# Elensil/Facet_Graph_Convolution

Measured on AMD Instinct MI355X. Metric: facets/sec (fwd+bwd) on 100k-facet mesh, higher is better.
Workload: dtype f32; 1 GPU; c2: torus 250x200 quads = 100000 facets per GPU (N0=122224 padded nodes), full graph U-Net + MLP: rotate + forward + angular loss + backward + Adam, fp32, hipGraph replay; parallelism=single GPU

## Files before the change

### facet_graph_convolution_amd/csrc/fgc_conv_bwd.hip

```cpp
#include <stdio.h>
#include <stdlib.h>
#include <string.h>

#include <algorithm>
#include <type_traits>

#include "fgc_conv_bwd.h"
#include "fgc_conv_narrow.h"
#include "fgc_conv_pair.h"
#include "fgc_gemm_tn.h"
#include "fgc_reduce.h"
#include "fgc_split.h"

namespace fgc {

__device__ __forceinline__ float slope_from_y(float y, float alpha) { return y > 0.f ? 1.f : (y < 0.f ? alpha : 0.f); }

__device__ __forceinline__ float pool4_grad_term(const float* __restrict__ y, const float* __restrict__ pool_y,
                                                 const float* __restrict__ pool_dy, int r, int col, int cout, int bf16) {
    const size_t pi = (size_t)(r >> 2) * cout + col;
    const float m = ld_act(pool_y, pi, bf16);
    const size_t b = (size_t)(r & ~3) * cout + col;
    float ne = 0.f;
#pragma unroll
// ... 752 lines not shown
                    }
                    dq[n0 + nn] += t0 + t1;
                }
            };
            products(0, bxa);
            if (!LONG) {
                products(H, bxb);
            } else {
                gather(H, bxa);
                products(H, bxa);
#pragma unroll
                for (int nn = 0; nn < NPW; ++nn) {
                    if (dn[nn] <= 16) continue;
                    const int node = wave * NPW + nn;
                    const int e = min(16 + lr, dn[nn] - 1);
                    const int row = __float_as_int(s.qbuf[(size_t)node * qnode_stride(QS) + e * QLD + 9]);
                    const unsigned off = __umul24((unsigned)row, rowbytes) + laneoff;
                    const f32x4 x0 = __builtin_bit_cast(f32x4, __builtin_amdgcn_raw_buffer_load_b128(rsrc, off, 0, 0));
                    const f32x4 x1 = __builtin_bit_cast(f32x4, __builtin_amdgcn_raw_buffer_load_b128(rsrc, off + 64u, 0, 0));
                    const float* zr = s.ztile + (size_t)node * ZSTRIDE + mrow * KC + 4 * lq;
                    const f32x4 a0 = *reinterpret_cast<const f32x4*>(zr);
                    const f32x4 a1 = *reinterpret_cast<const f32x4*>(zr + 16);
                    f32x4 u0 = f32x4{0.f, 0.f, 0.f, 0.f}, u1 = f32x4{0.f, 0.f, 0.f, 0.f};
#pragma unroll
                    for (int t = 0; t < 4; ++t) {
                        u0 = __builtin_amdgcn_mfma_f32_16x16x4f32(a0[t], x0[t], u0, 0, 0, 0);
                        u1 = __builtin_amdgcn_mfma_f32_16x16x4f32(a1[t], x1[t], u1, 0, 0, 0);
                    }
                    dq_hi[nn] += u0 + u1;
                }
            }
        }

#pragma unroll
        for (int nn = 0; nn < NPW; ++nn) {
            const int node = wave * NPW + nn;
            const int i = tile0 + node;
            const int d = dn[nn];
            if (i >= p.n) continue;
            if (d <= ebase) {
                if (sweep == 0 && lr == 0 && lq < 3)
                    *reinterpret_cast<f32x4*>(lp.dag + (size_t)i * FGC_AG_LD + 4 * lq) = f32x4{0.f, 0.f, 0.f, 0.f};
                continue;
            }
            const int e0 = s.deg[TILE + 4 + node];
            f32x4 da = f32x4{0.f, 0.f, 0.f, 0.f};
            const int ntile = (FGC_KO1 & 32) ? 0 : ((LONG && d > 16) ? 2 : 1);
            for (int et = 0; et < ntile; ++et) {
                const int edge = ebase + 16 * et + lr;
                const bool ok = edge < d;
                const float* qr = s.qbuf + (size_t)node * qnode_stride(QS) + min(edge, d - 1) * QLD;
                f32x4 q = f32x4{0.f, 0.f, 0.f, 0.f};
                if (lq < 2) q = *reinterpret_cast<const f32x4*>(qr + 4 * lq);
                else if (lq == 2) q[0] = qr[8];
                f32x4 g = (LONG && et == 1) ? dq_hi[LONG ? nn : 0] : dq[nn];
                if (lq == 2) { g[1] = 0.f; g[2] = 0.f; g[3] = 0.f; }
                if (lq == 3) g = f32x4{0.f, 0.f, 0.f, 0.f};
                float dot = q[0] * g[0] + q[1] * g[1] + q[2] * g[2] + q[3] * g[3];
                dot += __shfl_xor(dot, 16);
                dot += __shfl_xor(dot, 32);
                f32x4 dl;
#pragma unroll
                for (int t = 0; t < 4; ++t) dl[t] = ok ? q[t] * (g[t] - dot) : 0.f;
                if (!(FGC_KO1 & 64) && ok && lq < 3) *reinterpret_cast<f32x4*>(lp.dl + (size_t)(e0 + edge) * FGC_DL_LD + 4 * lq) = dl;
                da += dl;
            }
// ... 977 lines not shown
```

### facet_graph_convolution_amd/csrc/fgc_conv_w8.hip

```cpp
#include <stdlib.h>

#include "fgc_conv_w8.h"

namespace fgc {

#ifndef FGC_KO
#define FGC_KO 0
#endif
constexpr int W8_THREADS = 512;
constexpr int W8_LPN = 16;
typedef float f32x2 __attribute__((ext_vector_type(2)));

__device__ __forceinline__ f32x2 load_chunk2(const CoreParams& p, int row, int cbase) {
    const float* ptr = cbase < p.c0 ? p.src0 + (size_t)row * p.c0 + cbase
                                    : p.src1 + (size_t)row * p.c1 + (cbase - p.c0);
    f32x2 v = {0.f, 0.f};
    if (cbase < p.cg) v = *reinterpret_cast<const f32x2*>(ptr);
    return v;
}

template <int N, bool BF>
__device__ __forceinline__ void edge_batch(__amdgpu_buffer_rsrc_t rsrc, unsigned rowbytes, unsigned laneoff,
                                           const float* qk, f32x2 (&z)[FGC_M]) {
    f32x2 q89[N], xv[N];
// ... 27 lines not shown
#pragma unroll
    for (int t = 0; t < N; ++t) rid[t] = (unsigned)__float_as_int(qb[(T0 + t) * QLD + 9]);
#pragma unroll
    for (int t = 0; t < N; ++t) {
        const unsigned off = __umul24(rid[t], rowbytes) + laneoff;
        if (FGC_KO & 16) { raw[T0 + t] = f32x2{__uint_as_float(off), 1.f}; continue; }
        if constexpr (BF) raw[T0 + t][0] = __builtin_bit_cast(float, __builtin_amdgcn_raw_buffer_load_b32(rsrc, off, 0, 0));
        else raw[T0 + t] = __builtin_bit_cast(f32x2, __builtin_amdgcn_raw_buffer_load_b64(rsrc, off, 0, 0));
    }
}
template <int T0, int N, bool BF>
__device__ __forceinline__ void fma_rows(const float* qb, const f32x2 (&raw)[16], f32x2 (&z)[FGC_M]) {
#pragma unroll
    for (int t = 0; t < N; ++t) {
        const float* qk = qb + (T0 + t) * QLD;
        f32x2 xv;
        if constexpr (BF) xv = bf2_to_f2(__builtin_bit_cast(unsigned, raw[T0 + t][0]));
        else xv = raw[T0 + t];
        if (FGC_KO & 2) { z[t % FGC_M] += xv; continue; }
        const f32x4 q0 = *reinterpret_cast<const f32x4*>(qk);
        const f32x4 q1 = *reinterpret_cast<const f32x4*>(qk + 4);
        const float q8 = qk[8];
        z[0] += q0[0] * xv; z[1] += q0[1] * xv; z[2] += q0[2] * xv; z[3] += q0[3] * xv;
        z[4] += q1[0] * xv; z[5] += q1[1] * xv; z[6] += q1[2] * xv; z[7] += q1[3] * xv;
        z[8] += q8 * xv;
    }
}
__device__ __forceinline__ void wave_lds_sync() {
    __builtin_amdgcn_fence(__ATOMIC_RELEASE, "wavefront");
    __builtin_amdgcn_wave_barrier();
    __builtin_amdgcn_fence(__ATOMIC_ACQUIRE, "wavefront");
}

template <bool DATA, bool FAST, int QS, bool BF = false, int NT = 32, bool EROW = false>
__global__ __launch_bounds__(NT * 16, 4) void conv_w8_kernel(CoreParams p, FwdEpilogue fe, DataEpilogue de) {
    static_assert(!BF || FAST, "the bf16 form exists for the fast shapes only");
    static_assert(!EROW || (DATA && FAST), "rows by edge id: the data-gradient kernel's fast shapes");
    static_assert(NT == 32 || (NT == 16 && FAST && QS == 16), "half tiles: the pipelined 16-slot form only");
    constexpr int TILE = NT, RT = NT / 16, NW = NT / 4, LW = NT == 32 ? 3 : 2, W8_THREADS = NT * 16;
    extern __shared__ __attribute__((aligned(16))) char smem_raw[];
    const Smem s = carve(smem_raw, BF ? ZSTRIDE_BF / 2 : ZSTRIDE, QS, NT);
    constexpr int SPL = QS / 16 + (QS % 16 ? 1 : 0);
    constexpr bool PIPE = FAST && QS == 16;
    auto dag_slot = [&](int nd, int m) { return s.qbuf + (size_t)nd * qnode_stride(QS) + m * QLD + 10; };
    int tile0;
    if constexpr (NT == 32) {
        tile0 = block_tile0(p);
    } else {
        const int h = xcd_tile(blockIdx.x, gridDim.x);
        tile0 = (p.tile_list ? p.tile_list[h >> 1] : (h >> 1)) * 32 + (h & 1) * 16;
    }
    const int tid = threadIdx.x;
    const int node = tid >> 4, kl = tid & 15;
    const int wave = tid >> 6, lane = tid & 63, lr = lane & 15, lq = lane >> 4;
    const int nct = p.npad >> 4;
    const int nsh = 31 - __builtin_clz(nct);
    const int kparts = NW >> nsh;
    const int ct = __builtin_amdgcn_readfirstlane(wave & (nct - 1));
    const int kpart = __builtin_amdgcn_readfirstlane(wave >> nsh);
    constexpr int UPP = BF ? KPASS / 32 : KPASS / 16;
    const int u0 = __builtin_amdgcn_readfirstlane((UPP * kpart) >> (LW - nsh));
    const int u1 = __builtin_amdgcn_readfirstlane((UPP * (kpart + 1)) >> (LW - nsh));
    const __amdgpu_buffer_rsrc_t w_rs = __builtin_amdgcn_make_buffer_rsrc(const_cast<float*>(p.Wp), 0, -1, 0x00020000);
    const unsigned w_lane = BF ? (unsigned)((ct * 64 + lane) * 16) : (unsigned)((lq * p.npad + ct * 16 + lr) * 16);
    const unsigned w_unit = BF ? (unsigned)(nct * 1024) : (unsigned)(p.npad * 64);
    auto loadw = [&](int pass, int u) {
        const int uu = min(u, u1 - 1);
        if (FGC_KO & 512) return u32x4{(unsigned)uu, (unsigned)pass, 0x3f800000u, 0x3f000000u};
        return __builtin_bit_cast(u32x4, __builtin_amdgcn_raw_buffer_load_b128(w_rs, w_lane, (unsigned)(pass * UPP + uu) * w_unit, 0));
    };
    f32x2 xa[16];
    const float* qb = s.qbuf + (size_t)node * qnode_stride(QS);
    auto issue = [&](int pass, int dw) {
        constexpr unsigned ESZ = BF ? 2u : 4u;
        const bool first = pass * KC < p.c0;
        const float* base = first ? p.src0 : p.src1;
// ... 109 lines not shown
#pragma unroll
            for (int m = 0; m < FGC_M; ++m) {
                l[m] = __builtin_amdgcn_exp2f(fmaf(l[m], 1.4426950408889634f, nmx));
                sum += l[m];
            }
            const float inv = 1.0f / sum;
            float* q = s.qbuf + (size_t)node * qnode_stride(QS) + k * QLD;
            *reinterpret_cast<f32x4*>(q) = f32x4{l[0] * inv, l[1] * inv, l[2] * inv, l[3] * inv};
            *reinterpret_cast<f32x4*>(q + 4) = f32x4{l[4] * inv, l[5] * inv, l[6] * inv, l[7] * inv};
            q[8] = l[8] * inv;
            if (!PIPE) q[9] = __int_as_float(er[t]);
            if (DATA && !(FGC_KO & 256)) {
                const __amdgpu_buffer_rsrc_t dl_rs = __builtin_amdgcn_make_buffer_rsrc(const_cast<float*>(de.dl), 0, -1, 0x00020000);
                const unsigned dof = __umul24((unsigned)(EROW ? er[t] : p.eid[e0 + k]), FGC_DL_LD * 4u);
                const f32x4 d0 = __builtin_bit_cast(f32x4, __builtin_amdgcn_raw_buffer_load_b128(dl_rs, dof, 0, 0));
                const f32x4 d1 = __builtin_bit_cast(f32x4, __builtin_amdgcn_raw_buffer_load_b128(dl_rs, dof + 16u, 0, 0));
                dgsum[0] += d0[0]; dgsum[1] += d0[1]; dgsum[2] += d0[2]; dgsum[3] += d0[3];
                dgsum[4] += d1[0]; dgsum[5] += d1[1]; dgsum[6] += d1[2]; dgsum[7] += d1[3];
                dgsum[8] += __builtin_bit_cast(float, __builtin_amdgcn_raw_buffer_load_b32(dl_rs, dof + 32u, 0, 0));
            }
        }
        if (DATA) {
#pragma unroll
            for (int m = 0; m < FGC_M; ++m) {
                float v = dgsum[m];
                FGC_ROW16_SUM(v);
                dgsum[m] = v;
            }
            if (kl == 0) {
                if (i < p.n) {
                    const float da[FGC_M] = {da0[0], da0[1], da0[2], da0[3], da1[0], da1[1], da1[2], da1[3], da8};
#pragma unroll
                    for (int m = 0; m < FGC_M; ++m) *reinterpret_cast<f32x2*>(dag_slot(node, m)) = f32x2{da[m], dgsum[m]};
                    float* o = de.dag + (size_t)i * FGC_AG_LD + 12;
                    *reinterpret_cast<f32x4*>(o) = f32x4{dgsum[0], dgsum[1], dgsum[2], dgsum[3]};
                    *reinterpret_cast<f32x4*>(o + 4) = f32x4{dgsum[4], dgsum[5], dgsum[6], dgsum[7]};
                    *reinterpret_cast<f32x4*>(o + 8) = f32x4{dgsum[8], 0.f, 0.f, 0.f};
                    if constexpr (BF) {
                        u32x2* rt = reinterpret_cast<u32x2*>(reinterpret_cast<unsigned short*>(de.r) + (size_t)i * de.rld +
                                                             (FGC_M * p.cg));
                        rt[0] = f4_to_bf4(f32x4{da[0], da[1], da[2], da[3]});
                        rt[1] = f4_to_bf4(f32x4{da[4], da[5], da[6], da[7]});
                        rt[2] = f4_to_bf4(f32x4{da[8], 0.f, 0.f, 0.f});
                        rt[3] = f4_to_bf4(f32x4{dgsum[0], dgsum[1], dgsum[2], dgsum[3]});
                        rt[4] = f4_to_bf4(f32x4{dgsum[4], dgsum[5], dgsum[6], dgsum[7]});
                        rt[5] = f4_to_bf4(f32x4{dgsum[8], 0.f, 0.f, 0.f});
                    } else {
                    float* rt = de.r + (size_t)i * de.rld + (FGC_M * p.cg);
                    *reinterpret_cast<f32x4*>(rt) = f32x4{da[0], da[1], da[2], da[3]};
                    *reinterpret_cast<f32x4*>(rt + 4) = f32x4{da[4], da[5], da[6], da[7]};
                    *reinterpret_cast<f32x4*>(rt + 8) = f32x4{da[8], 0.f, 0.f, 0.f};
                    *reinterpret_cast<f32x4*>(rt + 12) = f32x4{dgsum[0], dgsum[1], dgsum[2], dgsum[3]};
                    *reinterpret_cast<f32x4*>(rt + 16) = f32x4{dgsum[4], dgsum[5], dgsum[6], dgsum[7]};
                    *reinterpret_cast<f32x4*>(rt + 20) = f32x4{dgsum[8], 0.f, 0.f, 0.f};
                    }
                }
            }
        }
    }
    if constexpr (PIPE) wave_lds_sync();
    else __syncthreads();

    f32x4 acc[RT];
#pragma unroll
    for (int r = 0; r < RT; ++r) acc[r] = f32x4{0.f, 0.f, 0.f, 0.f};
    const bool want_gemm = !DATA || de.dx0 != nullptr;

    const int cl = kl;
    const int d = s.deg[node];
    auto do_pass = [&](int pass) {
        f32x2 z[FGC_M];
#pragma unroll
        for (int m = 0; m < FGC_M; ++m) z[m] = f32x2{0.f, 0.f};
        const int cbase = pass * KC + 2 * cl;
        if constexpr (PIPE) {
            fma_rows<0, 8, BF>(qb, xa, z);
            if (dwave > 8) fma_rows<8, 4, BF>(qb, xa, z);
            if (dwave > 12) fma_rows<12, 1, BF>(qb, xa, z);
            if (dwave > 13) fma_rows<13, 1, BF>(qb, xa, z);
            if (dwave > 14) fma_rows<14, 2, BF>(qb, xa, z);
            if (pass + 1 < p.passes) issue(pass + 1, dwave);
        } else if (FAST) {
            const bool first = pass * KC < p.c0;
            const float* base = first ? p.src0 : p.src1;
            constexpr unsigned ESZ = BF ? 2u : 4u;
            const unsigned rowbytes = (unsigned)(first ? p.c0 : p.c1) * ESZ;
            const unsigned laneoff = (unsigned)(first ? cbase : cbase - p.c0) * ESZ;
            const __amdgpu_buffer_rsrc_t rsrc = __builtin_amdgcn_make_buffer_rsrc(const_cast<float*>(base), 0, -1, 0x00020000);
            int k0 = 0;
            for (; k0 + 8 <= dwave; k0 += 8) edge_batch<8, BF>(rsrc, rowbytes, laneoff, qb + k0 * QLD, z);
            const int rem = dwave - k0;
            if (rem > 4) {
                if (rem > 6) edge_batch<8, BF>(rsrc, rowbytes, laneoff, qb + k0 * QLD, z);
                else edge_batch<6, BF>(rsrc, rowbytes, laneoff, qb + k0 * QLD, z);
            } else if (rem > 0) {
                if (rem > 2) edge_batch<4, BF>(rsrc, rowbytes, laneoff, qb + k0 * QLD, z);
                else edge_batch<2, BF>(rsrc, rowbytes, laneoff, qb + k0 * QLD, z);
            }
        } else
        for (int k0 = 0; k0 < d; k0 += RB) {
            f32x2 xv[RB];
#pragma unroll
            for (int t = 0; t < RB; ++t) {
                xv[t] = f32x2{0.f, 0.f};
                if (k0 + t < d) xv[t] = load_chunk2(p, __float_as_int(qb[(k0 + t) * QLD + 9]), cbase);
            }
#pragma unroll
            for (int t = 0; t < RB; ++t) {
                if (k0 + t < d) {
                    const float* q = qb + (k0 + t) * QLD;
                    const f32x4 q0 = *reinterpret_cast<const f32x4*>(q);
                    const f32x4 q1 = *reinterpret_cast<const f32x4*>(q + 4);
                    const float q8 = q[8];
                    z[0] += q0[0] * xv[t]; z[1] += q0[1] * xv[t]; z[2] += q0[2] * xv[t]; z[3] += q0[3] * xv[t];
                    z[4] += q1[0] * xv[t]; z[5] += q1[1] * xv[t]; z[6] += q1[2] * xv[t]; z[7] += q1[3] * xv[t];
                    z[8] += q8 * xv[t];
                }
            }
        }        if (DATA) {
            const int j = tile0 + node;
            if (!(FGC_KO & 128) && j < p.n && cbase < p.cg) {
                if constexpr (BF) {
                    unsigned* rr = reinterpret_cast<unsigned*>(reinterpret_cast<unsigned short*>(de.r) + (size_t)j * de.rld + cbase);
#pragma unroll
                    for (int m = 0; m < FGC_M; ++m) rr[(m * p.cg) >> 1] = f2_to_bf2(z[m][0], z[m][1]);
                } else {
                float* rr = de.r + (size_t)j * de.rld + cbase;
#pragma unroll
                for (int m = 0; m < FGC_M; ++m) *reinterpret_cast<f32x2*>(rr + m * p.cg) = z[m];
                }
            }
            if (!want_gemm) return;
        }
        auto gphase32 = [&](int gl, int gh, int gz) {
        auto loadw = [&](int pass_, int u) {
            const int uu = min(u, gh - 1);
            if (FGC_KO & 512) return u32x4{(unsigned)uu, (unsigned)pass_, 0x3f800000u, 0x3f000000u};
            return __builtin_bit_cast(u32x4, __builtin_amdgcn_raw_buffer_load_b128(w_rs, w_lane, (unsigned)(pass_ * UPP + uu) * w_unit, 0));
        };
        auto loada = [&](int g, f32x4 (&a)[RT]) {
            const int gg = min(g, gh - 1) - gz;
#pragma unroll
            for (int r = 0; r < RT; ++r)
                a[r] = *reinterpret_cast<const f32x4*>(s.ztile + (size_t)(r * 16 + lr) * ZSTRIDE + gg * 16 + lq * 4);
        };
        auto mm = [&](const f32x4 (&a)[RT], const u32x4& bw) {
            const f32x4 b = __builtin_bit_cast(f32x4, bw);
#pragma unroll
            for (int t = 0; t < 4; ++t)
#pragma unroll
                for (int r = 0; r < RT; ++r) {
                    if (FGC_KO & 1) asm volatile("" ::"v"(a[r][t]), "v"(b[t]));
// ... 9 lines not shown
                mm(a0, b0);
                b0 = loadw(pass, g + 4);
                loada(g + 2, a0);
                mm(a1, b1);
                b1 = loadw(pass, g + 5);
                loada(g + 3, a1);
                mm(a0, b2);
                b2 = loadw(pass, g + 6);
                loada(g + 4, a0);
                mm(a1, b3);
                b3 = loadw(pass, g + 7);
            }
            if (g < gh) {
                loada(g + 1, a1);
                mm(a0, b0);
            }
            if (g + 1 < gh) {
                loada(g + 2, a0);
                mm(a1, b1);
            }
            if (g + 2 < gh) mm(a0, b2);
        };
        if (pass > 0) __syncthreads();
        if constexpr (BF) {
            unsigned* zr = reinterpret_cast<unsigned*>(s.ztile) + (size_t)node * (ZSTRIDE_BF / 2) + cl;
#pragma unroll
            for (int m = 0; m < FGC_M; ++m) zr[m * (KC / 2)] = f2_to_bf2(z[m][0], z[m][1]);
        } else {
            float* zr = s.ztile + (size_t)node * ZSTRIDE + 2 * cl;
#pragma unroll
            for (int m = 0; m < FGC_M; ++m) *reinterpret_cast<f32x2*>(zr + m * KC) = z[m];
        }
        __syncthreads();
        if (FGC_KO & 8) return;
        const char* zb = reinterpret_cast<const char*>(s.ztile);
        auto mmb = [&](int ks, const u32x4& b) {
#pragma unroll
            for (int r = 0; r < RT; ++r) {
                const u32x4 a = *reinterpret_cast<const u32x4*>(zb + (size_t)(r * 16 + lr) * (ZSTRIDE_BF * 2) + ks * 64 + lq * 16);
                acc[r] = __builtin_amdgcn_mfma_f32_16x16x32_bf16(__builtin_bit_cast(bf16x8, a), __builtin_bit_cast(bf16x8, b),
                                                                acc[r], 0, 0, 0);
            }
        };
        if constexpr (BF) {
            int ks = u0;
            u32x4 b0 = loadw(pass, ks), b1 = loadw(pass, ks + 1);
            for (; ks + 2 <= u1; ks += 2) {
                mmb(ks, b0);
                b0 = loadw(pass, ks + 2);
                mmb(ks + 1, b1);
                b1 = loadw(pass, ks + 3);
            }
            if (ks < u1) mmb(ks, b0);
        } else {
            gphase32(u0, u1, 0);
        }
    };
    for (int pass = 0; pass < p.passes; ++pass) do_pass(pass);
    if (!want_gemm) return;
    if (FGC_KO & 32) { if (acc[0][0] == 123.f && acc[RT - 1][3] == 5.f) s.ztile[tid] = acc[0][1]; return; }
    __syncthreads();
    const int oldd = p.npad + 4;
    float* otile = s.ztile;
    {
        float* base = otile + (size_t)kpart * TILE * oldd;
#pragma unroll
        for (int r = 0; r < RT; ++r)
#pragma unroll
            for (int t = 0; t < 4; ++t) base[(size_t)(r * 16 + lq * 4 + t) * oldd + ct * 16 + lr] = acc[r][t];
    }
    __syncthreads();
    if (!DATA) {
        const int osh = 31 - __builtin_clz(p.nout);
        const bool pow2 = FAST && (p.nout & (p.nout - 1)) == 0;
        const int o = pow2 ? (tid & (p.nout - 1)) : tid % p.nout, pstep = pow2 ? (W8_THREADS >> osh) : W8_THREADS / p.nout;
        const float bias_o = fe.bias[o];
        for (int pr = tid < pstep * p.nout ? (pow2 ? tid >> osh : tid / p.nout) : TILE; pr < TILE / 4; pr += pstep) {
            float mx = -INFINITY;
            bool any = false;
            const size_t ybase = (size_t)(tile0 + pr * 4) * p.nout + o;
#pragma unroll
            for (int q = 0; q < 4; ++q) {
                const int row = pr * 4 + q;
                const int i = tile0 + row;
                if (i >= p.n) continue;
                float val = 0.f;
                for (int kp = 0; kp < kparts; ++kp) val += otile[((size_t)kp * TILE + row) * oldd + o];
                const int dd = s.deg[row];
                val *= __int_as_float(s.deg[TILE + 4 + row]);
                if (!fe.bias_mask || dd > 0) val += bias_o;
                if (fe.act) val = fmaxf(val, 0.f) - fe.alpha * fmaxf(-val, 0.f);
                st_act(fe.y, ybase + (size_t)(q * p.nout), val, BF);
// ... 11 lines not shown
        float uc[FGC_M], vc[FGC_M];
#pragma unroll
        for (int m = 0; m < FGC_M; ++m) {
            uc[m] = de.u[m * de.cin + c];
            vc[m] = de.v[m * de.cin + c];
        }
        for (int sr = tid < sstep * de.cin ? (pow2 ? tid >> csh : tid / de.cin) : nsrc; sr < nsrc; sr += sstep) {
            float val = 0.f;
            bool any = false;
            for (int q = 0; q < group; ++q) {
                const int row = sr * group + q;
                if (tile0 + row >= p.n) continue;
                any = true;
                float g = 0.f;
                for (int kp = 0; kp < kparts; ++kp) g += otile[((size_t)kp * TILE + row) * oldd + c];
#pragma unroll
                for (int m = 0; m < FGC_M; ++m) {
                    const f32x2 dd = *reinterpret_cast<const f32x2*>(dag_slot(row, m));
                    g = fmaf(dd[0], uc[m], g);
                    g = fmaf(dd[1], vc[m], g);
                }
                val += g;
            }
            if (!any) continue;
            const size_t srow = (size_t)((tile0 >> de.shiftf) + sr);
            if (c < de.c0f) {
                const size_t o = srow * de.c0f + c;
                st_act(de.dx0, o, de.acc0 ? ld_act(de.dx0, o, BF) + val : val, BF);
            } else if (de.dx1) {
                const size_t o = srow * de.c1f + (c - de.c0f);
                st_act(de.dx1, o, de.acc1 ? ld_act(de.dx1, o, BF) + val : val, BF);
            }
        }
    }
}

bool w8_supported(const CoreParams& p, int max_deg) {
    if (opt(OPT_NO_W8) == 1) return false;
    const int nct = p.npad >> 4;
    if (!(nct == 1 || nct == 2 || nct == 4 || nct == 8)) return false;
    if (max_deg <= 0 || max_deg > KMAX) return false;
    if (p.kc != 32) return false;
    if ((p.c0 & 1) || (p.c1 & 1)) return false;
    if (((uintptr_t)p.src0 & 7) || (p.src1 && ((uintptr_t)p.src1 & 7))) return false;
    return true;
}

static bool w8_fast(const CoreParams& p) {
    if (opt(OPT_NO_W8FAST) == 1) return false;
    return p.cg % 32 == 0 && (p.c1 == 0 || p.c0 % 32 == 0) && (size_t)p.n * 4 * 128 < 0xFFFFFFFFull;
}

static bool w8_half_tiles(const CoreParams& p, bool data) {
    const int mode = (int)opt(OPT_W8_NT16), min_n = (int)opt(OPT_W8_DATA16_MIN_N);
    if ((p.npad >> 4) > 4 || mode < 1) return false;
    return !data || mode >= 2 || p.n >= min_n;
}

template <bool DATA, bool FAST, int QS, bool BF = false, bool EROW = false>
static int launch_w8f(const CoreParams& p, const FwdEpilogue& fe, const DataEpilogue& de, size_t smem, const W8Form& f,
                      hipStream_t st) {
    static bool attr = false;
    if (!attr) {
        hipFuncSetAttribute((const void*)conv_w8_kernel<DATA, FAST, QS, BF, 32, EROW>, hipFuncAttributeMaxDynamicSharedMemorySize,
                            160 * 1024);
        attr = true;
    }
    if constexpr (FAST && QS == 16) {
        if (f.nt == 16) {
            constexpr int NT = 16;
            const size_t zrow = BF ? (size_t)ZSTRIDE_BF * 2 : (size_t)ZSTRIDE * 4;
            size_t smem16 = NT * zrow + (size_t)NT * qnode_stride(16) * 4 + (2 * NT + 4) * 4 + 64;
            if (DATA) smem16 += (size_t)opt(OPT_W8_DATA_SMEM_PAD);
            FGC_LAUNCH(DATA ? "conv_w8_kernel<data>" : "conv_w8_kernel<fwd>", st, (conv_w8_kernel<DATA, FAST, QS, BF, NT, EROW>),
                       dim3(2 * core_grid(p)), dim3(NT * 16), smem16, p, fe, de);
            FGC_CHECK_LAUNCH("conv_w8_kernel (half tiles)");
            return FGC_OK;
        }
    }
    smem -= (size_t)TILE * (qnode_stride(KMAX) - qnode_stride(QS)) * 4;
    if (BF) smem -= (size_t)TILE * (ZSTRIDE * 4 - ZSTRIDE_BF * 2);
    FGC_LAUNCH(DATA ? "conv_w8_kernel<data>" : "conv_w8_kernel<fwd>", st, (conv_w8_kernel<DATA, FAST, QS, BF, 32, EROW>),
               dim3(core_grid(p)), dim3(W8_THREADS), smem, p, fe, de);
    FGC_CHECK_LAUNCH("conv_w8_kernel");
    return FGC_OK;
}

bool w8_bf16_supported(const CoreParams& p, int max_deg) {
    const int nct = p.npad >> 4;
    return w8_supported(p, max_deg) && w8_fast(p) && (nct == 2 || nct == 4 || nct == 8) && p.nout == p.npad;
}

static bool bfm_r_ok(const DataEpilogue& de) { return ((uintptr_t)de.r & 15) == 0 && de.rld % 8 == 0; }

W8Form w8_form(const CoreParams& p, const DataEpilogue* de, int max_deg, bool bf16) {
    W8Form f;
    const bool data = de != nullptr;
    f.bfm = bf16 && bfm_supported(p, max_deg, data, data ? de->cin : 0) && (!data || bfm_r_ok(*de));
    f.fast = bf16 || w8_fast(p);
    f.qs = (f.fast && max_deg <= 16) ? 16 : KMAX;
    f.nt = ((f.bfm || (f.fast && f.qs == 16)) && w8_half_tiles(p, data)) ? 16 : TILE;
    return f;
}

template <bool DATA>
static int launch_w8(const CoreParams& p, const FwdEpilogue& fe, const DataEpilogue& de, size_t smem, int max_deg,
                     bool bf16, hipStream_t st) {
    const W8Form f = w8_form(p, DATA ? &de : nullptr, max_deg, bf16);
    if (f.bfm) return DATA ? launch_data_bfm(p, de, f.nt == 16, false, st) : launch_fwd_bfm(p, fe, f.nt == 16, st);
    if (bf16)
        return f.qs == 16 ? launch_w8f<DATA, true, 16, true>(p, fe, de, smem, f, st)
                          : launch_w8f<DATA, true, KMAX, true>(p, fe, de, smem, f, st);
    if (!f.fast) return launch_w8f<DATA, false, KMAX>(p, fe, de, smem, f, st);
    return f.qs == 16 ? launch_w8f<DATA, true, 16>(p, fe, de, smem, f, st)
                      : launch_w8f<DATA, true, KMAX>(p, fe, de, smem, f, st);
}

int launch_fwd_w8(const CoreParams& p, const FwdEpilogue& ep, size_t smem, int max_deg, hipStream_t st, bool bf16) {
// ... 21 lines not shown
```

### facet_graph_convolution_amd/csrc/fgc_mlp_split.hip

```cpp
#include "fgc_mlp.h"
#include "fgc_mlp_mb.h"
#include "fgc_split.h"

namespace fgc {

template <int KS, int CO>
__global__ __launch_bounds__(MB_THREADS, 2) void mlp_fwd_split_kernel(const float* __restrict__ x, int n, int hidden, int cout,
                                                                      const u32x4* __restrict__ Wp16,
                                                                      const float* __restrict__ b1,
                                                                      const float* __restrict__ W2,
                                                                      const float* __restrict__ b2, float alpha,
                                                                      float* __restrict__ y, float* __restrict__ abs_partial) {
    __shared__ float ypart[4 * MB_FWD_T * 4];
    __shared__ float red[4];
    constexpr int CIN = KS * 32;
    const int row0 = blockIdx.x * MB_FWD_T;
    const int wave = threadIdx.x >> 6, lane = threadIdx.x & 63, lr = lane & 15, lq = lane >> 4;
    const int nct = hidden >> 4;
    const size_t plane = (size_t)KS * nct * 64;
    u32x4 a[MB_FWD_RT][KS][3];
#pragma unroll
    for (int r = 0; r < MB_FWD_RT; ++r) {
        const int row = min(row0 + r * 16 + lr, n - 1);
#pragma unroll
        for (int ks = 0; ks < KS; ++ks) {
            const f32x4* src = reinterpret_cast<const f32x4*>(x + (size_t)row * CIN + ks * 32 + 8 * lq);
            u32x2 lo[3], hi[3];
            split3(src[0], lo[0], lo[1], lo[2]);
            split3(src[1], hi[0], hi[1], hi[2]);
#pragma unroll
            for (int p = 0; p < 3; ++p) a[r][ks][p] = u32x4{lo[p][0], lo[p][1], hi[p][0], hi[p][1]};
        }
    }
    float yp[MB_FWD_RT][4][CO];
#pragma unroll
    for (int r = 0; r < MB_FWD_RT; ++r)
#pragma unroll
        for (int t = 0; t < 4; ++t)
#pragma unroll
            for (int o = 0; o < CO; ++o) yp[r][t][o] = 0.f;

    u32x4 bnext[KS][3];
    float bbn = 0.f, w2n[CO];
    auto fetch_weights = [&](int ct) {
        ct = min(ct, nct - 1);
#pragma unroll
        for (int ks = 0; ks < KS; ++ks)
#pragma unroll
            for (int p = 0; p < 3; ++p) bnext[ks][p] = Wp16[p * plane + ((size_t)ks * nct + ct) * 64 + lane];
        bbn = b1[ct * 16 + lr];
#pragma unroll
        for (int o = 0; o < CO; ++o) w2n[o] = W2[(size_t)(ct * 16 + lr) * cout + min(o, cout - 1)];
    };
    fetch_weights(wave);
    for (int ct = wave; ct < nct; ct += 4) {
        u32x4 bcur[KS][3];
        float w2[CO];
#pragma unroll
        for (int ks = 0; ks < KS; ++ks)
#pragma unroll
            for (int p = 0; p < 3; ++p) bcur[ks][p] = bnext[ks][p];
        const float bb = bbn;
#pragma unroll
        for (int o = 0; o < CO; ++o) w2[o] = o < cout ? w2n[o] : 0.f;
        fetch_weights(ct + 4);
        f32x4 h[MB_FWD_RT];
#pragma unroll
        for (int r = 0; r < MB_FWD_RT; ++r) h[r] = f32x4{bb, bb, bb, bb};
#pragma unroll
        for (int ks = 0; ks < KS; ++ks)
#pragma unroll
            for (int r = 0; r < MB_FWD_RT; ++r) h[r] = mfma_split(a[r][ks], bcur[ks], h[r]);
#pragma unroll
        for (int r = 0; r < MB_FWD_RT; ++r)
#pragma unroll
            for (int t = 0; t < 4; ++t) {
                float v = h[r][t];
                v = lrelu01(v, alpha);
#pragma unroll
                for (int o = 0; o < CO; ++o) yp[r][t][o] = fmaf(v, w2[o], yp[r][t][o]);
            }
    }
#pragma unroll
    for (int r = 0; r < MB_FWD_RT; ++r)
#pragma unroll
        for (int t = 0; t < 4; ++t)
#pragma unroll
            for (int o = 0; o < CO; ++o) {
                float v = yp[r][t][o];
                FGC_ROW16_SUM(v);
                yp[r][t][o] = v;
            }
    if (lr == 0) {
#pragma unroll
        for (int r = 0; r < MB_FWD_RT; ++r)
#pragma unroll
            for (int t = 0; t < 4; ++t)
#pragma unroll
                for (int o = 0; o < CO; ++o) ypart[(wave * MB_FWD_T + r * 16 + lq * 4 + t) * 4 + o] = yp[r][t][o];
    }
    __syncthreads();
    float asum = 0.f;
    for (int t = threadIdx.x; t < MB_FWD_T * cout; t += MB_THREADS) {
        const int r = t / cout, o = t % cout;
        const int row = row0 + r;
        if (row < n) {
            float v = b2[o];
            v += ypart[(0 * MB_FWD_T + r) * 4 + o];
            v += ypart[(1 * MB_FWD_T + r) * 4 + o];
            v += ypart[(2 * MB_FWD_T + r) * 4 + o];
            v += ypart[(3 * MB_FWD_T + r) * 4 + o];
            y[(size_t)row * cout + o] = v;
            asum += fabsf(v);
        }
// ... 237 lines not shown
        request(min(tile + nwalkers, ntiles - 1));
        __builtin_amdgcn_sched_barrier(0);
        u32x4 gA[MB_RT];
#pragma unroll
        for (int r = 0; r < MB_RT; ++r) {
            const u32x4 f = *reinterpret_cast<const u32x4*>(t + MB_T * XTS + MB_T * 16 + (r * 16 + lr) * 48 + min(lq, 2) * 16);
            const unsigned keep = lq < 3 ? ~0u : 0u;
            gA[r] = u32x4{f[0] & keep, f[1] & keep, f[2] & keep, f[3] & keep};
        }
        u32x4 ax[MB_RT][KS][3];
#pragma unroll
        for (int r = 0; r < MB_RT; ++r)
#pragma unroll
            for (int ks = 0; ks < KS; ++ks)
#pragma unroll
                for (int p = 0; p < 3; ++p)
                    ax[r][ks][p] = *reinterpret_cast<const u32x4*>(t + (r * 16 + lr) * XTS + p * XPL + (ks * 32 + 8 * lq) * 2);
        u32x4 af[MT][3];
#pragma unroll
        for (int m = 0; m < MT; ++m)
#pragma unroll
            for (int p = 0; p < 3; ++p) af[m][p] = mbs_xT_frag(t + p * XPL, XTS, m * 16, lq, lr);
        if (blockIdx.y == 0 && wave == 0 && lr == 0) {
#pragma unroll
            for (int j = 0; j < 8; ++j) {
                const f32x4 d = *reinterpret_cast<const f32x4*>(dyw + ((j >> 2) * 16 + 4 * lq + (j & 3)) * 4);
#pragma unroll
                for (int o = 0; o < 3; ++o) db2acc[o] += d[o];
            }
        }
#pragma unroll
        for (int c = 0; c < MBW_CT; ++c) {
            __builtin_amdgcn_sched_barrier(0);
            asm volatile("" ::: "memory");
            f32x4 h[MB_RT], g[MB_RT];
#pragma unroll
            for (int r = 0; r < MB_RT; ++r) h[r] = f32x4{bb[c], bb[c], bb[c], bb[c]};
#pragma unroll
            for (int ks = 0; ks < KS; ++ks)
#pragma unroll
                for (int r = 0; r < MB_RT; ++r) h[r] = mfma_split(ax[r][ks], bw[c][ks], h[r]);
#pragma unroll
            for (int r = 0; r < MB_RT; ++r)
                g[r] = __builtin_amdgcn_mfma_f32_16x16x32_bf16(__builtin_bit_cast(bf16x8, gA[r]), __builtin_bit_cast(bf16x8, bg[c]),
                                                              f32x4{0.f, 0.f, 0.f, 0.f}, 0, 0, 0);
            __builtin_amdgcn_sched_barrier(0);
#pragma unroll
            for (int r = 0; r < MB_RT; ++r)
#pragma unroll
                for (int t4 = 0; t4 < 4; ++t4) {
                    const f32x4 dyv = *reinterpret_cast<const f32x4*>(dyw + (r * 16 + 4 * lq + t4) * 4);
                    const float pre = h[r][t4];
                    const float slope = lrelu01_slope(pre, alpha);
                    const float ha = pre * slope;
                    g[r][t4] *= slope;
                    db1acc[c] += g[r][t4];
#pragma unroll
                    for (int o = 0; o < 3; ++o) dW2acc[c][o] = fmaf(ha, dyv[o], dW2acc[c][o]);
                }
            u32x4 bf[3];
            split3_frag(g[0], g[1], bf);
            __builtin_amdgcn_sched_barrier(0);
#pragma unroll
            for (int m = 0; m < MT; ++m) {
                dW1acc[c][m] = mfma_split(af[m], bf, dW1acc[c][m]);
                asm volatile("" : "+v"(dW1acc[c][m])::"memory");
            }
// ... 72 lines not shown
```

Before: 63.44 million facets/s.

## Defer data-gradient row stores, specialize pass count, double-buffer MLP weight fetches

In the w8 data-gradient kernel's pipelined fp32 form, the per-pass scattered writes of the r matrix and the dag/r tail rows move out of the FMA phase. They are now done as coalesced buffer stores from the LDS z-tile after each pass and after the epilogue, and the pass count becomes a template parameter so the pass loop can unroll. The MLP forward kernel gets a two-slot ping-pong weight prefetch using buffer loads and scheduling barriers. The backward conv kernel gains an explicit waitcnt, and an asm memory clobber is replaced by a sched_barrier. The aim is to overlap global latency with MFMA work and cut uncoalesced stores, at the cost of more template instances and extra register pressure.

```diff
diff --git a/facet_graph_convolution_amd/csrc/fgc_conv_bwd.hip b/facet_graph_convolution_amd/csrc/fgc_conv_bwd.hip
--- a/facet_graph_convolution_amd/csrc/fgc_conv_bwd.hip
+++ b/facet_graph_convolution_amd/csrc/fgc_conv_bwd.hip
@@ -808,6 +808,7 @@
             }
         }
 
+        __builtin_amdgcn_s_waitcnt(0x0F70);
 #pragma unroll
         for (int nn = 0; nn < NPW; ++nn) {
             const int node = wave * NPW + nn;
diff --git a/facet_graph_convolution_amd/csrc/fgc_conv_w8.hip b/facet_graph_convolution_amd/csrc/fgc_conv_w8.hip
--- a/facet_graph_convolution_amd/csrc/fgc_conv_w8.hip
+++ b/facet_graph_convolution_amd/csrc/fgc_conv_w8.hip
@@ -83,7 +83,7 @@
     __builtin_amdgcn_fence(__ATOMIC_ACQUIRE, "wavefront");
 }
 
-template <bool DATA, bool FAST, int QS, bool BF = false, int NT = 32, bool EROW = false>
+template <bool DATA, bool FAST, int QS, bool BF = false, int NT = 32, bool EROW = false, int NP = 0>
 __global__ __launch_bounds__(NT * 16, 4) void conv_w8_kernel(CoreParams p, FwdEpilogue fe, DataEpilogue de) {
     static_assert(!BF || FAST, "the bf16 form exists for the fast shapes only");
     static_assert(!EROW || (DATA && FAST), "rows by edge id: the data-gradient kernel's fast shapes");
@@ -93,6 +93,8 @@
     const Smem s = carve(smem_raw, BF ? ZSTRIDE_BF / 2 : ZSTRIDE, QS, NT);
     constexpr int SPL = QS / 16 + (QS % 16 ? 1 : 0);
     constexpr bool PIPE = FAST && QS == 16;
+    constexpr bool RLATE = DATA && PIPE && !BF;
+    static_assert(NP == 0 || RLATE, "a compile-time pass count: the late-store form only");
     auto dag_slot = [&](int nd, int m) { return s.qbuf + (size_t)nd * qnode_stride(QS) + m * QLD + 10; };
     int tile0;
     if constexpr (NT == 32) {
@@ -268,27 +270,29 @@
                     const float da[FGC_M] = {da0[0], da0[1], da0[2], da0[3], da1[0], da1[1], da1[2], da1[3], da8};
 #pragma unroll
                     for (int m = 0; m < FGC_M; ++m) *reinterpret_cast<f32x2*>(dag_slot(node, m)) = f32x2{da[m], dgsum[m]};
-                    float* o = de.dag + (size_t)i * FGC_AG_LD + 12;
-                    *reinterpret_cast<f32x4*>(o) = f32x4{dgsum[0], dgsum[1], dgsum[2], dgsum[3]};
-                    *reinterpret_cast<f32x4*>(o + 4) = f32x4{dgsum[4], dgsum[5], dgsum[6], dgsum[7]};
-                    *reinterpret_cast<f32x4*>(o + 8) = f32x4{dgsum[8], 0.f, 0.f, 0.f};
-                    if constexpr (BF) {
-                        u32x2* rt = reinterpret_cast<u32x2*>(reinterpret_cast<unsigned short*>(de.r) + (size_t)i * de.rld +
-                                                             (FGC_M * p.cg));
-                        rt[0] = f4_to_bf4(f32x4{da[0], da[1], da[2], da[3]});
-                        rt[1] = f4_to_bf4(f32x4{da[4], da[5], da[6], da[7]});
-                        rt[2] = f4_to_bf4(f32x4{da[8], 0.f, 0.f, 0.f});
-                        rt[3] = f4_to_bf4(f32x4{dgsum[0], dgsum[1], dgsum[2], dgsum[3]});
-                        rt[4] = f4_to_bf4(f32x4{dgsum[4], dgsum[5], dgsum[6], dgsum[7]});
-                        rt[5] = f4_to_bf4(f32x4{dgsum[8], 0.f, 0.f, 0.f});
-                    } else {
-                    float* rt = de.r + (size_t)i * de.rld + (FGC_M * p.cg);
-                    *reinterpret_cast<f32x4*>(rt) = f32x4{da[0], da[1], da[2], da[3]};
-                    *reinterpret_cast<f32x4*>(rt + 4) = f32x4{da[4], da[5], da[6], da[7]};
-                    *reinterpret_cast<f32x4*>(rt + 8) = f32x4{da[8], 0.f, 0.f, 0.f};
-                    *reinterpret_cast<f32x4*>(rt + 12) = f32x4{dgsum[0], dgsum[1], dgsum[2], dgsum[3]};
-                    *reinterpret_cast<f32x4*>(rt + 16) = f32x4{dgsum[4], dgsum[5], dgsum[6], dgsum[7]};
-                    *reinterpret_cast<f32x4*>(rt + 20) = f32x4{dgsum[8], 0.f, 0.f, 0.f};
+                    if constexpr (!RLATE) {
+                        float* o = de.dag + (size_t)i * FGC_AG_LD + 12;
+                        *reinterpret_cast<f32x4*>(o) = f32x4{dgsum[0], dgsum[1], dgsum[2], dgsum[3]};
+                        *reinterpret_cast<f32x4*>(o + 4) = f32x4{dgsum[4], dgsum[5], dgsum[6], dgsum[7]};
+                        *reinterpret_cast<f32x4*>(o + 8) = f32x4{dgsum[8], 0.f, 0.f, 0.f};
+                        if constexpr (BF) {
+                            u32x2* rt = reinterpret_cast<u32x2*>(reinterpret_cast<unsigned short*>(de.r) + (size_t)i * de.rld +
+                                                                 (FGC_M * p.cg));
+                            rt[0] = f4_to_bf4(f32x4{da[0], da[1], da[2], da[3]});
+                            rt[1] = f4_to_bf4(f32x4{da[4], da[5], da[6], da[7]});
+                            rt[2] = f4_to_bf4(f32x4{da[8], 0.f, 0.f, 0.f});
+                            rt[3] = f4_to_bf4(f32x4{dgsum[0], dgsum[1], dgsum[2], dgsum[3]});
+                            rt[4] = f4_to_bf4(f32x4{dgsum[4], dgsum[5], dgsum[6], dgsum[7]});
+                            rt[5] = f4_to_bf4(f32x4{dgsum[8], 0.f, 0.f, 0.f});
+                        } else {
+                        float* rt = de.r + (size_t)i * de.rld + (FGC_M * p.cg);
+                        *reinterpret_cast<f32x4*>(rt) = f32x4{da[0], da[1], da[2], da[3]};
+                        *reinterpret_cast<f32x4*>(rt + 4) = f32x4{da[4], da[5], da[6], da[7]};
+                        *reinterpret_cast<f32x4*>(rt + 8) = f32x4{da[8], 0.f, 0.f, 0.f};
+                        *reinterpret_cast<f32x4*>(rt + 12) = f32x4{dgsum[0], dgsum[1], dgsum[2], dgsum[3]};
+                        *reinterpret_cast<f32x4*>(rt + 16) = f32x4{dgsum[4], dgsum[5], dgsum[6], dgsum[7]};
+                        *reinterpret_cast<f32x4*>(rt + 20) = f32x4{dgsum[8], 0.f, 0.f, 0.f};
+                        }
                     }
                 }
             }
@@ -304,6 +308,48 @@
 
     const int cl = kl;
     const int d = s.deg[node];
+    const int npasses = NP > 0 ? NP : p.passes;
+    int rhi = 0;
+    const float* rz = nullptr;
+    unsigned r_off = 0;
+    __amdgpu_buffer_rsrc_t r_rs = w_rs;
+    if constexpr (RLATE) {
+        const int rnode = (tid >> 3) & (TILE - 1);
+        rhi = tid >> (LW + 5);
+        rz = s.ztile + (size_t)rnode * ZSTRIDE + rhi * KC + (tid & 7) * 4;
+        const int t0 = __builtin_amdgcn_readfirstlane(tile0);
+        const int rows = __builtin_amdgcn_readfirstlane(max(min(p.n - t0, TILE), 0));
+        r_rs = __builtin_amdgcn_make_buffer_rsrc(de.r + (size_t)t0 * de.rld, 0, rows * de.rld * 4, 0x00020000);
+        r_off = (unsigned)(rnode * de.rld + rhi * p.cg + (tid & 7) * 4) * 4u;
+    }
+    auto store_r = [&](int pass) {
+        if constexpr (RLATE) {
+            if (FGC_KO & 128) return;
+            f32x4 v[5];
+#pragma unroll
+            for (int t = 0; t < 5; ++t) v[t] = *reinterpret_cast<const f32x4*>(rz + 2 * t * KC);
+            const unsigned pc = (unsigned)(pass * KC) * 4u, mstep = (unsigned)p.cg * 8u;
+#pragma unroll
+            for (int t = 0; t < 5; ++t) {
+                const unsigned off = (t == 4 && rhi) ? 0x80000000u : r_off + t * mstep;
+                __builtin_amdgcn_raw_buffer_store_b128(__builtin_bit_cast(u32x4, v[t]), r_rs, off, pc, 0);
+            }
+        }
+    };
+    auto store_dag_rows = [&]() {
+        if constexpr (RLATE) {
+            const int i = tile0 + node;
+            if (kl < 9 && i < p.n) {
+                const int q = kl % 3;
+                const float* sl = dag_slot(node, 4 * q) + (kl >= 3 ? 1 : 0);
+                const float v1 = sl[QLD], v2 = sl[2 * QLD], v3 = sl[3 * QLD];
+                const f32x4 v = {sl[0], q < 2 ? v1 : 0.f, q < 2 ? v2 : 0.f, q < 2 ? v3 : 0.f};
+                float* o = kl < 6 ? de.r + (size_t)i * de.rld + (FGC_M * p.cg) + kl * 4
+                                  : de.dag + (size_t)i * FGC_AG_LD + 12 + (kl - 6) * 4;
+                *reinterpret_cast<f32x4*>(o) = v;
+            }
+        }
+    };
     auto do_pass = [&](int pass) {
         f32x2 z[FGC_M];
 #pragma unroll
@@ -315,7 +361,7 @@
             if (dwave > 12) fma_rows<12, 1, BF>(qb, xa, z);
             if (dwave > 13) fma_rows<13, 1, BF>(qb, xa, z);
             if (dwave > 14) fma_rows<14, 2, BF>(qb, xa, z);
-            if (pass + 1 < p.passes) issue(pass + 1, dwave);
+            if (pass + 1 < npasses) issue(pass + 1, dwave);
         } else if (FAST) {
             const bool first = pass * KC < p.c0;
             const float* base = first ? p.src0 : p.src1;
@@ -353,7 +399,8 @@
                     z[8] += q8 * xv[t];
                 }
             }
-        }        if (DATA) {
+        }
+        if (DATA && !RLATE) {
             const int j = tile0 + node;
             if (!(FGC_KO & 128) && j < p.n && cbase < p.cg) {
                 if constexpr (BF) {
@@ -429,7 +476,8 @@
             for (int m = 0; m < FGC_M; ++m) *reinterpret_cast<f32x2*>(zr + m * KC) = z[m];
         }
         __syncthreads();
-        if (FGC_KO & 8) return;
+        if (RLATE && !want_gemm) { store_r(pass); return; }
+        if (FGC_KO & 8) { store_r(pass); return; }
         const char* zb = reinterpret_cast<const char*>(s.ztile);
         auto mmb = [&](int ks, const u32x4& b) {
 #pragma unroll
@@ -452,9 +500,15 @@
         } else {
             gphase32(u0, u1, 0);
         }
+        store_r(pass);
     };
-    for (int pass = 0; pass < p.passes; ++pass) do_pass(pass);
-    if (!want_gemm) return;
+    if constexpr (NP > 0) {
+#pragma unroll
+        for (int pass = 0; pass < NP; ++pass) do_pass(pass);
+    } else {
+        for (int pass = 0; pass < p.passes; ++pass) do_pass(pass);
+    }
+    if (!want_gemm) { store_dag_rows(); return; }
     if (FGC_KO & 32) { if (acc[0][0] == 123.f && acc[RT - 1][3] == 5.f) s.ztile[tid] = acc[0][1]; return; }
     __syncthreads();
     const int oldd = p.npad + 4;
@@ -532,6 +586,7 @@
                 st_act(de.dx1, o, de.acc1 ? ld_act(de.dx1, o, BF) + val : val, BF);
             }
         }
+        store_dag_rows();
     }
 }
 
@@ -557,12 +612,12 @@
     return !data || mode >= 2 || p.n >= min_n;
 }
 
-template <bool DATA, bool FAST, int QS, bool BF = false, bool EROW = false>
-static int launch_w8f(const CoreParams& p, const FwdEpilogue& fe, const DataEpilogue& de, size_t smem, const W8Form& f,
+template <bool DATA, bool FAST, int QS, bool BF, bool EROW, int NP>
+static int launch_w8n(const CoreParams& p, const FwdEpilogue& fe, const DataEpilogue& de, size_t smem, const W8Form& f,
                       hipStream_t st) {
     static bool attr = false;
     if (!attr) {
-        hipFuncSetAttribute((const void*)conv_w8_kernel<DATA, FAST, QS, BF, 32, EROW>, hipFuncAttributeMaxDynamicSharedMemorySize,
+        hipFuncSetAttribute((const void*)conv_w8_kernel<DATA, FAST, QS, BF, 32, EROW, NP>, hipFuncAttributeMaxDynamicSharedMemorySize,
                             160 * 1024);
         attr = true;
     }
@@ -572,7 +627,7 @@
             const size_t zrow = BF ? (size_t)ZSTRIDE_BF * 2 : (size_t)ZSTRIDE * 4;
             size_t smem16 = NT * zrow + (size_t)NT * qnode_stride(16) * 4 + (2 * NT + 4) * 4 + 64;
             if (DATA) smem16 += (size_t)opt(OPT_W8_DATA_SMEM_PAD);
-            FGC_LAUNCH(DATA ? "conv_w8_kernel<data>" : "conv_w8_kernel<fwd>", st, (conv_w8_kernel<DATA, FAST, QS, BF, NT, EROW>),
+            FGC_LAUNCH(DATA ? "conv_w8_kernel<data>" : "conv_w8_kernel<fwd>", st, (conv_w8_kernel<DATA, FAST, QS, BF, NT, EROW, NP>),
                        dim3(2 * core_grid(p)), dim3(NT * 16), smem16, p, fe, de);
             FGC_CHECK_LAUNCH("conv_w8_kernel (half tiles)");
             return FGC_OK;
@@ -580,10 +635,21 @@
     }
     smem -= (size_t)TILE * (qnode_stride(KMAX) - qnode_stride(QS)) * 4;
     if (BF) smem -= (size_t)TILE * (ZSTRIDE * 4 - ZSTRIDE_BF * 2);
-    FGC_LAUNCH(DATA ? "conv_w8_kernel<data>" : "conv_w8_kernel<fwd>", st, (conv_w8_kernel<DATA, FAST, QS, BF, 32, EROW>),
+    FGC_LAUNCH(DATA ? "conv_w8_kernel<data>" : "conv_w8_kernel<fwd>", st, (conv_w8_kernel<DATA, FAST, QS, BF, 32, EROW, NP>),
                dim3(core_grid(p)), dim3(W8_THREADS), smem, p, fe, de);
     FGC_CHECK_LAUNCH("conv_w8_kernel");
     return FGC_OK;
+}
+
+template <bool DATA, bool FAST, int QS, bool BF = false, bool EROW = false>
+static int launch_w8f(const CoreParams& p, const FwdEpilogue& fe, const DataEpilogue& de, size_t smem, const W8Form& f,
+                      hipStream_t st) {
+    if constexpr (DATA && FAST && QS == 16 && !BF) {
+        if (p.passes == 1) return launch_w8n<DATA, FAST, QS, BF, EROW, 1>(p, fe, de, smem, f, st);
+        if (p.passes == 2) return launch_w8n<DATA, FAST, QS, BF, EROW, 2>(p, fe, de, smem, f, st);
+        if (p.passes == 4) return launch_w8n<DATA, FAST, QS, BF, EROW, 4>(p, fe, de, smem, f, st);
+    }
+    return launch_w8n<DATA, FAST, QS, BF, EROW, 0>(p, fe, de, smem, f, st);
 }
 
 bool w8_bf16_supported(const CoreParams& p, int max_deg) {
diff --git a/facet_graph_convolution_amd/csrc/fgc_mlp_split.hip b/facet_graph_convolution_amd/csrc/fgc_mlp_split.hip
--- a/facet_graph_convolution_amd/csrc/fgc_mlp_split.hip
+++ b/facet_graph_convolution_amd/csrc/fgc_mlp_split.hip
@@ -40,46 +40,67 @@
 #pragma unroll
             for (int o = 0; o < CO; ++o) yp[r][t][o] = 0.f;
 
-    u32x4 bnext[KS][3];
-    float bbn = 0.f, w2n[CO];
-    auto fetch_weights = [&](int ct) {
-        ct = min(ct, nct - 1);
+    const int wv = __builtin_amdgcn_readfirstlane(wave);
+    const __amdgpu_buffer_rsrc_t wp_rs = __builtin_amdgcn_make_buffer_rsrc(const_cast<u32x4*>(Wp16), 0, (int)(3 * plane * 16), 0x00020000);
+    const __amdgpu_buffer_rsrc_t b1_rs = __builtin_amdgcn_make_buffer_rsrc(const_cast<float*>(b1), 0, hidden * 4, 0x00020000);
+    const __amdgpu_buffer_rsrc_t w2_rs = __builtin_amdgcn_make_buffer_rsrc(const_cast<float*>(W2), 0, hidden * cout * 4, 0x00020000);
+    const unsigned wp_lane = (unsigned)lane * 16u, b1_lane = (unsigned)lr * 4u, w2_lane = (unsigned)(lr * cout) * 4u;
+    struct Tile {
+        u32x4 b[KS][3];
+        float bb, w2[CO];
+    };
+    auto fetch = [&](Tile& t, int ct) {
+        const unsigned c = (unsigned)min(ct, nct - 1);
 #pragma unroll
         for (int ks = 0; ks < KS; ++ks)
 #pragma unroll
-            for (int p = 0; p < 3; ++p) bnext[ks][p] = Wp16[p * plane + ((size_t)ks * nct + ct) * 64 + lane];
-        bbn = b1[ct * 16 + lr];
-#pragma unroll
-        for (int o = 0; o < CO; ++o) w2n[o] = W2[(size_t)(ct * 16 + lr) * cout + min(o, cout - 1)];
-    };
-    fetch_weights(wave);
-    for (int ct = wave; ct < nct; ct += 4) {
-        u32x4 bcur[KS][3];
+            for (int p = 0; p < 3; ++p)
+                t.b[ks][p] = __builtin_bit_cast(u32x4, __builtin_amdgcn_raw_buffer_load_b128(
+                    wp_rs, wp_lane, (unsigned)((p * plane + ((size_t)ks * nct + c) * 64) * 16), 0));
+        t.bb = __builtin_bit_cast(float, __builtin_amdgcn_raw_buffer_load_b32(b1_rs, b1_lane, c * 64u, 0));
+#pragma unroll
+        for (int o = 0; o < CO; ++o)
+            t.w2[o] = __builtin_bit_cast(float, __builtin_amdgcn_raw_buffer_load_b32(
+                w2_rs, w2_lane, (c * 16u * (unsigned)cout + (unsigned)min(o, cout - 1)) * 4u, 0));
+    };
+    auto tile = [&](const Tile& t) {
         float w2[CO];
 #pragma unroll
+        for (int o = 0; o < CO; ++o) w2[o] = o < cout ? t.w2[o] : 0.f;
+        f32x4 h[MB_FWD_RT];
+#pragma unroll
+        for (int r = 0; r < MB_FWD_RT; ++r) h[r] = f32x4{t.bb, t.bb, t.bb, t.bb};
+#pragma unroll
         for (int ks = 0; ks < KS; ++ks)
 #pragma unroll
-            for (int p = 0; p < 3; ++p) bcur[ks][p] = bnext[ks][p];
-        const float bb = bbn;
-#pragma unroll
-        for (int o = 0; o < CO; ++o) w2[o] = o < cout ? w2n[o] : 0.f;
-        fetch_weights(ct + 4);
-        f32x4 h[MB_FWD_RT];
-#pragma unroll
-        for (int r = 0; r < MB_FWD_RT; ++r) h[r] = f32x4{bb, bb, bb, bb};
-#pragma unroll
-        for (int ks = 0; ks < KS; ++ks)
-#pragma unroll
-            for (int r = 0; r < MB_FWD_RT; ++r) h[r] = mfma_split(a[r][ks], bcur[ks], h[r]);
+            for (int r = 0; r < MB_FWD_RT; ++r) h[r] = mfma_split(a[r][ks], t.b[ks], h[r]);
 #pragma unroll
         for (int r = 0; r < MB_FWD_RT; ++r)
 #pragma unroll
-            for (int t = 0; t < 4; ++t) {
-                float v = h[r][t];
+            for (int t4 = 0; t4 < 4; ++t4) {
+                float v = h[r][t4];
                 v = lrelu01(v, alpha);
 #pragma unroll
-                for (int o = 0; o < CO; ++o) yp[r][t][o] = fmaf(v, w2[o], yp[r][t][o]);
+                for (int o = 0; o < CO; ++o) yp[r][t4][o] = fmaf(v, w2[o], yp[r][t4][o]);
             }
+    };
+    Tile ta, tb;
+    int ct = wv;
+    fetch(ta, ct);
+    if (((nct - wv + 3) >> 2) & 1) {
+        tile(ta);
+        ct += 4;
+        fetch(ta, ct);
+    }
+    for (; ct < nct; ct += 8) {
+        fetch(tb, ct + 4);
+        __builtin_amdgcn_sched_barrier(0);
+        tile(ta);
+        __builtin_amdgcn_sched_barrier(0);
+        fetch(ta, ct + 8);
+        __builtin_amdgcn_sched_barrier(0);
+        tile(tb);
+        __builtin_amdgcn_sched_barrier(0);
     }
 #pragma unroll
     for (int r = 0; r < MB_FWD_RT; ++r)
@@ -383,7 +404,7 @@
 #pragma unroll
         for (int c = 0; c < MBW_CT; ++c) {
             __builtin_amdgcn_sched_barrier(0);
-            asm volatile("" ::: "memory");
+            __builtin_amdgcn_sched_barrier(0);
             f32x4 h[MB_RT], g[MB_RT];
 #pragma unroll
             for (int r = 0; r < MB_RT; ++r) h[r] = f32x4{bb[c], bb[c], bb[c], bb[c]};
```

Result: no change. 63.83 million facets/s, median of 6 (+0.6%).
